# jcmgray/cotengra

Hardware: NVIDIA H100
Metric: sycamore_n53_m20_sliced_contract_tflops (higher is better)
Workload: dtype c128 (f64 arithmetic)

## Files before the change

cotengra_b200/_lib.py:

```python

from __future__ import annotations

import ctypes as C
import os

from . import lowering

_HERE = os.path.dirname(os.path.abspath(__file__))
LIB_PATH = os.path.join(_HERE, "libctgb200.so")

EXPORTS = (
    "ctgb_abi_version",
    "ctgb_desc_words",
    "ctgb_single_desc_words",
    "ctgb_last_error",
    "ctgb_device_info",
    "ctgb_contract_pair",
    "ctgb_reduce_single",
    "ctgb_plan_create",
    "ctgb_plan_set_chunk_desc",
    "ctgb_plan_set_scale_slots",
    "ctgb_plan_destroy",
    "ctgb_plan_workspace_bytes",
    "ctgb_plan_launches_per_slice",
    "ctgb_plan_strip_modes",
    "ctgb_plan_execute",
    "ctgb_plan_execute_host",
    "ctgb_launch_count",
    "ctgb_tensor_map_launches",
    "ctgb_plan_profile",
    "ctgb_plan_profile_read",
    "ctgb_probe_fp64_peaks",
    "ctgb_tc05_launch_config",
    "ctgb_dmmastream_launch_config",
)
TC05_LAUNCH_FIELDS = ("b_stat", "nb", "sa", "grid", "smem", "tm_rank", "bulk", "chunk_steps", "chunks")
DMMASTREAM_LAUNCH_FIELDS = ("nj", "rows", "grid")


class CtgbTensor(C.Structure):
    _fields_ = [
        ("kind", C.c_int32),
        ("input_index", C.c_int32),
        ("offset", C.c_int64),
        ("nbytes", C.c_int64),
        ("n_sliced", C.c_int32),
        ("slice_pos", C.POINTER(C.c_int32)),
        ("slice_stride", C.POINTER(C.c_int64)),
    ]


class CtgbNode(C.Structure):
    _fields_ = [
        ("kind", C.c_int32),
        ("a", C.c_int32),
        ("b", C.c_int32),
        ("c", C.c_int32),
        ("phase", C.c_int32),
        ("zero_fill", C.c_int32),
        ("is_root", C.c_int32),
# ... 53 lines not shown
    ]
    lib.ctgb_contract_pair.argtypes = [C.c_void_p] * 5
    lib.ctgb_reduce_single.argtypes = [C.c_void_p] * 4
    lib.ctgb_plan_create.argtypes = [C.POINTER(CtgbPlanDesc), C.POINTER(C.c_void_p)]
    lib.ctgb_plan_set_chunk_desc.argtypes = [C.c_void_p, C.c_void_p]
    lib.ctgb_plan_set_scale_slots.argtypes = [C.c_void_p, C.POINTER(C.c_int32), C.POINTER(C.c_int32), C.c_int]
    lib.ctgb_plan_destroy.argtypes = [C.c_void_p]
    lib.ctgb_plan_destroy.restype = None
    lib.ctgb_plan_execute.argtypes = [
        C.c_void_p, C.POINTER(C.c_void_p), C.c_void_p, C.c_void_p, C.c_void_p, C.POINTER(C.c_void_p),
        C.c_void_p, C.c_size_t, C.c_int64, C.c_int64, C.c_int64, C.c_void_p,
    ]
    lib.ctgb_plan_execute_host.argtypes = [
        C.c_void_p, C.POINTER(C.c_void_p), C.POINTER(C.c_int64), C.c_void_p,
        C.POINTER(C.c_double), C.c_void_p, C.c_size_t, C.c_int64, C.c_int64,
        C.c_int64, C.c_void_p,
    ]
    lib.ctgb_plan_profile.argtypes = [C.c_void_p, C.c_int]
    lib.ctgb_plan_profile_read.argtypes = [C.c_void_p, C.POINTER(C.c_float), C.c_int]
    lib.ctgb_probe_fp64_peaks.argtypes = [C.POINTER(C.c_double), C.POINTER(C.c_double), C.c_void_p]
    lib.ctgb_tc05_launch_config.argtypes = [C.c_void_p, C.c_uint64, C.c_int, C.c_uint64,
                                            C.POINTER(C.c_int64), C.c_int]
    lib.ctgb_dmmastream_launch_config.argtypes = [C.c_void_p, C.c_int, C.POINTER(C.c_int64), C.c_int]
    if lib.ctgb_abi_version() != 2:
        raise ImportError("libctgb200.so: ABI version mismatch")
    if lib.ctgb_desc_words() != lowering.DESC_WORDS:
        raise ImportError("libctgb200.so: pair descriptor layout mismatch")
    if lib.ctgb_single_desc_words() != lowering.SDESC_WORDS:
        raise ImportError("libctgb200.so: single descriptor layout mismatch")
    _lib = lib
    return lib


def check(rc):
    if rc:
        msg = load().ctgb_last_error().decode()
        raise _ERRORS.get(rc, RuntimeError)(f"ctgb error {rc}: {msg}")


def device_info():
    lib = load()
    sm, ma, mi, sh = C.c_int(), C.c_int(), C.c_int(), C.c_size_t()
    check(lib.ctgb_device_info(C.byref(sm), C.byref(ma), C.byref(mi), C.byref(sh)))
    return {"sm_count": sm.value, "cc": (ma.value, mi.value), "smem_optin": sh.value}


# ... 9 lines not shown


def tensor_map_launches() -> int:
    return int(load().ctgb_tensor_map_launches())


def tc05_launch_config(words, a_addr, sms, smem_optin) -> dict:
    import numpy as np

    w = np.ascontiguousarray(words, dtype=np.int64)
    out = (C.c_int64 * len(TC05_LAUNCH_FIELDS))()
    check(load().ctgb_tc05_launch_config(w.ctypes.data, int(a_addr), int(sms), int(smem_optin), out,
                                         len(TC05_LAUNCH_FIELDS)))
    return dict(zip(TC05_LAUNCH_FIELDS, (int(x) for x in out)))


def dmmastream_launch_config(words, sms) -> dict:
    import numpy as np

    w = np.ascontiguousarray(words, dtype=np.int64)
    out = (C.c_int64 * len(DMMASTREAM_LAUNCH_FIELDS))()
    check(load().ctgb_dmmastream_launch_config(w.ctypes.data, int(sms), out, len(DMMASTREAM_LAUNCH_FIELDS)))
    return dict(zip(DMMASTREAM_LAUNCH_FIELDS, (int(x) for x in out)))
```

cotengra_b200/csrc/ctg_b200.cu:

```cuda
#include <cuda.h>
#include <cuda_runtime.h>
#include <stdint.h>
#include <stdio.h>
#include <stdlib.h>
#include <string.h>

#include <algorithm>
#include <atomic>
#include <type_traits>
#include <string>
#include <vector>

#include "../../include/ctg_b200.h"
#include "gett_desc.h"
#include "gett_kernels.cuh"
#include "probe.cuh"

using namespace ctgb;

namespace {

thread_local std::string g_err;
std::atomic<int64_t> g_launches{0};

// ... 32 lines not shown
      cached_dev = dev;
      cudaMemPool_t pool;
      if (cudaDeviceGetDefaultMemPool(&pool, dev) == cudaSuccess) {
        uint64_t keep = UINT64_MAX;
        cudaMemPoolSetAttribute(pool, cudaMemPoolAttrReleaseThreshold, &keep);
      }
    } else {
      d.ok = false;
    }
  }
  return d;
}

size_t elem_size(int dtype) {
  switch (dtype) {
    case CTGB_F32: return 4;
    case CTGB_F64: return 8;
    case CTGB_C64: return 8;
    case CTGB_C128: return 16;
  }
  return 0;
}

template <typename T, class P>
int launch_gett_policy(const int64_t* h, const int64_t* d, const void* A, const void* B, void* C, cudaStream_t st) {
  DevInfo& di = devinfo();
  if (!di.ok) return fail(CTGB_E_CUDA, "no CUDA device");
  constexpr size_t smem = GettSmem<P>::template bytes<T>();
  if (smem > di.smem_optin) return fail(CTGB_E_CUDA, "kernel variant needs more shared memory than the device offers");
  static thread_local int attr_dev = -1;
  int dev;
  cudaGetDevice(&dev);
  if (attr_dev != dev) {
    CUDA_TRY(cudaFuncSetAttribute(gett_kernel<T, P>, cudaFuncAttributeMaxDynamicSharedMemorySize, (int)smem));
    attr_dev = dev;
  }
  if constexpr (P::CONSUMER_REGS > 0) {
    static thread_local int checked = 0;
    if (!checked) {
      cudaFuncAttributes fa;
      CUDA_TRY(cudaFuncGetAttributes(&fa, gett_kernel<T, P>));
      const long pool = (long)fa.numRegs * (P::THREADS + PRODUCER_THREADS);
      const long want = (long)P::CONSUMER_REGS * P::THREADS + (long)P::PRODUCER_REGS * PRODUCER_THREADS;
      if (want > pool) return fail(CTGB_E_CUDA, "setmaxnreg budget exceeds the launch register pool");
      checked = 1;
    }
  }
  static thread_local int occ = 0;
  if (occ == 0) {
    CUDA_TRY(cudaOccupancyMaxActiveBlocksPerMultiprocessor(&occ, gett_kernel<T, P>, P::THREADS + PRODUCER_THREADS, smem));
    if (occ < 1) occ = 1;
  }
  const uint64_t work = (uint64_t)h[W_TILES_M] * (uint64_t)h[W_TILES_N] * (uint64_t)h[W_TILES_B] * (uint64_t)h[W_SPLITK];
  if (work == 0) return CTGB_OK;
  if (work >= (1ull << 31)) return fail(CTGB_E_VALUE, "too many tiles for one launch");
  uint64_t grid = (uint64_t)di.sms * occ;
  if (grid > work) grid = work;
  if (h[W_SPLITK] > 1 && !(h[W_FLAGS] & 1)) {
    if (h[W_CELEMS] <= 0) return fail(CTGB_E_VALUE, "split-K into a strided C needs accumulate");
    CUDA_TRY(cudaMemsetAsync(C, 0, (size_t)h[W_CELEMS] * sizeof(T), st));
  }
  gett_kernel<T, P><<<(unsigned)grid, P::THREADS + PRODUCER_THREADS, smem, st>>>(d, (const T*)A, (const T*)B, (T*)C);
  g_launches.fetch_add(1, std::memory_order_relaxed);
  CUDA_TRY(cudaGetLastError());
  return CTGB_OK;
}

template <typename T>
int launch_rowstream(const int64_t* h, const int64_t* d, const void* A, const void* B, void* C, cudaStream_t st) {
  DevInfo& di = devinfo();
  if (!di.ok) return fail(CTGB_E_CUDA, "no CUDA device");
  const int N = (int)h[W_NTA], K = (int)h[W_KTA];
  if (N > 8 || K > 8 || h[W_TILES_N] != 1 || h[W_TILES_B] != 1 || h[W_STEPS_K] != 1 || h[W_SPLITK] != 1 ||
      h[W_PGM] >= 0 && (h[W_MFULL] % h[W_MTEXT]) != 0 || h[W_PGN] >= 0 || h[W_PGK] >= 0)
    return fail(CTGB_E_VALUE, "descriptor does not fit the row-stream kernel");
  const unsigned long long M = (unsigned long long)h[W_MTA] * (unsigned long long)h[W_TILES_M];
  if (M >= (1ull << 32)) return fail(CTGB_E_VALUE, "too many rows for the row-stream kernel");
  unsigned long long blocks = (M + 255) / 256;
  const unsigned long long cap = (unsigned long long)di.sms * 8;
  if (blocks > cap) blocks = cap;
  if (blocks == 0) return CTGB_OK;
  const T* a = (const T*)A;
  const T* b = (const T*)B;
  T* c = (T*)C;
  const bool strip = h[W_SCALE_A] != 0 || h[W_FACTOR_C] != 0;
  if (N <= 4 && K <= 4) {
    if (strip) rowstream_kernel<T, 4, 4, true, true><<<(unsigned)blocks, 256, 0, st>>>(d, a, b, c);
    else rowstream_kernel<T, 4, 4, true><<<(unsigned)blocks, 256, 0, st>>>(d, a, b, c);
// ... 331 lines not shown

template <typename T>
int launch_gett_typed(const int64_t* h, const int64_t* d, const void* A, const void* B, void* C, cudaStream_t st) {
  const int variant = (int)h[W_VARIANT];
  const bool one = (h[W_FLAGS] & FLAG_TF32_ONE_PASS) != 0;
  if (variant == VAR_ROWSTREAM) return launch_rowstream<T>(h, d, A, B, C, st);
  if (variant == VAR_ROWSTREAM_K) return launch_rowstream_longk<T>(h, d, A, B, C, st);
  if (variant == VAR_DMMASTREAM) return launch_dmmastream(h, d, A, B, C, st);
  if (variant == VAR_DOTSTREAM || variant == VAR_DOTSTREAM4) return launch_dotstream<T>(h, d, A, B, C, st);
  if constexpr (std::is_same<T, float2>::value) {
    if (variant == VAR_TC05_128x64) return one ? launch_tc05<64, true>(h, d, A, B, C, st) : launch_tc05<64, false>(h, d, A, B, C, st);
    if (variant == VAR_TC05_128x32) return one ? launch_tc05<32, true>(h, d, A, B, C, st) : launch_tc05<32, false>(h, d, A, B, C, st);
    if (variant == VAR_TC05_128x16) return one ? launch_tc05<16, true>(h, d, A, B, C, st) : launch_tc05<16, false>(h, d, A, B, C, st);
  }
  switch (variant) {
    case VAR_SIMT_64x64: return launch_gett_policy<T, SimtPolicy<T, 64, 64, 8, 3>>(h, d, A, B, C, st);
    case VAR_KRED: return launch_gett_policy<T, KredPolicy<T, 1, 1, 512, 6>>(h, d, A, B, C, st);
    case VAR_ROW_128x8: return launch_gett_policy<T, RowPolicy<T, 256, 8, 4, 3>>(h, d, A, B, C, st);
    case VAR_ROW_256x4: return launch_gett_policy<T, RowPolicy<T, 256, 4, 4, 3>>(h, d, A, B, C, st);
    default: break;
  }
  if constexpr (sizeof(T) == 16 || (sizeof(T) == 8 && std::is_same<T, double>::value)) {
    switch (variant) {
      case VAR_DMMA_128x64: return launch_gett_policy<T, DmmaPolicy<T, 4, 2, 4, 4, 16, 3, false, 4>>(h, d, A, B, C, st);
      case VAR_DMMA_64x128: return launch_gett_policy<T, DmmaPolicy<T, 2, 4, 4, 4, 16, 3, false, 4>>(h, d, A, B, C, st);
      case VAR_DMMA_256x32: return launch_gett_policy<T, DmmaPolicy<T, 8, 1, 4, 4, 8, 4, false, 8>>(h, d, A, B, C, st);
      case VAR_DMMA_256x16: return launch_gett_policy<T, DmmaPolicy<T, 8, 1, 4, 2, 8, 5>>(h, d, A, B, C, st);
      case VAR_DMMA_32x32: return launch_gett_policy<T, DmmaPolicy<T, 2, 2, 2, 2, 16, 4>>(h, d, A, B, C, st);
      default: break;
    }
  }
  if constexpr (sizeof(T) == 16) {
    switch (variant) {
      case VAR_DMMA3M_128x32: return launch_gett_policy<T, DmmaPolicy<T, 4, 2, 4, 2, 16, 4, true>>(h, d, A, B, C, st);
      case VAR_DMMA3M_256x16: return launch_gett_policy<T, DmmaPolicy<T, 8, 1, 4, 2, 8, 5, true>>(h, d, A, B, C, st);
      default: break;
    }
  }
  if constexpr (std::is_same<T, float>::value || std::is_same<T, float2>::value) {
    switch (variant) {
#define CTGB_TF32(...)                                                                             \
  return one ? launch_gett_policy<T, Tf32Policy<T, __VA_ARGS__, true>>(h, d, A, B, C, st)           \
             : launch_gett_policy<T, Tf32Policy<T, __VA_ARGS__>>(h, d, A, B, C, st)
      case VAR_DMMA_128x64: CTGB_TF32(4, 2, 2, 4, 16, 3);
      case VAR_DMMA_64x128: CTGB_TF32(2, 4, 2, 4, 16, 3);
      case VAR_DMMA_256x32: CTGB_TF32(8, 1, 2, 4, 8, 3);
      case VAR_DMMA_256x16: CTGB_TF32(8, 1, 2, 2, 8, 3);
      case VAR_TF32_32x32: CTGB_TF32(2, 2, 1, 2, 16, 4);
#undef CTGB_TF32
      default: break;
    }
// ... 311 lines not shown
    default: return fail(CTGB_E_VALUE, "not a wgmma descriptor");
  }
  if (rc) return rc;
  const int64_t v[9] = {lc.b_stat, lc.nb, lc.sa, (int64_t)lc.grid, (int64_t)lc.smem, lc.tm_rank, lc.bulk,
                        (int64_t)lc.chunk, (int64_t)lc.chunks};
  for (int i = 0; i < 9; ++i) out[i] = v[i];
  return CTGB_OK;
}

int ctgb_dmmastream_launch_config(const int64_t* words, int sms, int64_t* out, int n_out) {
  if (!words || !out) return fail(CTGB_E_VALUE, "null argument");
  if (words[W_MAGIC] != DESC_MAGIC) return fail(CTGB_E_VALUE, "bad descriptor");
  if (n_out < 3) return fail(CTGB_E_VALUE, "ctgb_dmmastream_launch_config writes 3 words");
  if (sms < 1) return fail(CTGB_E_VALUE, "sms must be positive");
  if (words[W_VARIANT] != VAR_DMMASTREAM) return fail(CTGB_E_VALUE, "not a DMMA stream descriptor");
  DsLaunch lc;
  if (int rc = dmmastream_launch_config(words, sms, lc)) return rc;
  out[0] = lc.nj;
  out[1] = lc.rows;
  out[2] = (int64_t)lc.blocks;
  return CTGB_OK;
}

int ctgb_device_info(int* sm_count, int* cc_major, int* cc_minor, size_t* smem_optin_bytes) {
  DevInfo& d = devinfo();
  if (!d.ok) return fail(CTGB_E_CUDA, "no CUDA device");
  if (sm_count) *sm_count = d.sms;
  if (cc_major) *cc_major = d.major;
  if (cc_minor) *cc_minor = d.minor;
  if (smem_optin_bytes) *smem_optin_bytes = d.smem_optin;
  return CTGB_OK;
}

int ctgb_probe_fp64_peaks(double* dmma_tflops, double* dfma_tflops, void* stream) {
  DevInfo& di = devinfo();
  if (!di.ok) return fail(CTGB_E_CUDA, "no CUDA device");
  cudaStream_t st = (cudaStream_t)stream;
  double* sink = nullptr;
  CUDA_TRY(cudaMalloc((void**)&sink, 64));
  cudaEvent_t e0, e1;
  CUDA_TRY(cudaEventCreate(&e0));
  CUDA_TRY(cudaEventCreate(&e1));
  const int blocks = di.sms * 8, iters = 4096;
  auto timed = [&](int which, double flop_per_thread_iter, double* out) -> int {
    float best = 1e30f;
    for (int rep = 0; rep < 4; ++rep) {
// ... 412 lines not shown
```

cotengra_b200/csrc/gett_kernels.cuh:

```cuda
#pragma once
#include <cuda_runtime.h>
#include <math_constants.h>
#include <stdint.h>

#include <type_traits>

#include "gett_desc.h"

namespace ctgb {

__device__ __forceinline__ void mac(float& c, float a, float b) { c = fmaf(a, b, c); }
__device__ __forceinline__ void mac(double& c, double a, double b) { c = fma(a, b, c); }
__device__ __forceinline__ void mac(float2& c, float2 a, float2 b) {
  c.x = fmaf(a.x, b.x, c.x);
  c.x = fmaf(-a.y, b.y, c.x);
  c.y = fmaf(a.x, b.y, c.y);
  c.y = fmaf(a.y, b.x, c.y);
}
__device__ __forceinline__ void mac(double2& c, double2 a, double2 b) {
  c.x = fma(a.x, b.x, c.x);
  c.x = fma(-a.y, b.y, c.x);
  c.y = fma(a.x, b.y, c.y);
  c.y = fma(a.y, b.x, c.y);
}
// ... 381 lines not shown

template <typename T, int WARPS_M, int WARPS_N, int FM, int FN, int KT_, int STAGES_, bool M3_ = false,
          int B_SLOTS_ = STAGES_>
struct DmmaPolicy {
  static constexpr bool CPLX = sizeof(T) == 16;
  static constexpr bool M3 = M3_ && CPLX;
  static constexpr int MT = WARPS_M * FM * 8, NT = WARPS_N * FN * 8, KT = KT_, STAGES = STAGES_;
  static constexpr int THREADS = WARPS_M * WARPS_N * 32;
  static constexpr int A_ELEMS = MT * KT, B_ELEMS = NT * KT;
  static constexpr int B_SLOTS = B_SLOTS_;
  static constexpr int SCRATCH_ELEMS = 0;
  static constexpr int CONSUMER_REGS = (THREADS == 256) ? 232 : 0, PRODUCER_REGS = 40;
  static constexpr bool HAS_BCACHE = false;
  static constexpr int MIN_BLOCKS = THREADS <= 128 ? 2 : 1;
  static_assert(KT % 4 == 0, "KT must be a multiple of the DMMA k");
  static_assert(FM % 2 == 0, "real and 3M products issue one m16n8k4 DMMA per two 8-row fragments");
  static constexpr bool TR = CPLX && !M3;
  static constexpr bool SCAN_OK = true;
  struct Acc {
    double re[FM][FN][2];
    double im[CPLX ? FM : 1][CPLX ? FN : 1][2];
    double p3[M3 ? FM : 1][M3 ? FN : 1][2];
  };
  __device__ static __forceinline__ int idxA(int r, int kk) { return ((kk >> 2) * MT + r) * 4 + (kk & 3); }
  __device__ static __forceinline__ int idxB(int c, int kk) { return ((kk >> 2) * NT + c) * 4 + (kk & 3); }
  __device__ static __forceinline__ void clear(Acc& acc) {
#pragma unroll
    for (int i = 0; i < FM; ++i)
#pragma unroll
      for (int j = 0; j < FN; ++j) {
        acc.re[i][j][0] = acc.re[i][j][1] = 0.0;
        if constexpr (CPLX) acc.im[i][j][0] = acc.im[i][j][1] = 0.0;
        if constexpr (M3) acc.p3[i][j][0] = acc.p3[i][j][1] = 0.0;
      }
  }
  __device__ static __forceinline__ void compute(const T* __restrict__ sA, const T* __restrict__ sB, Acc& acc,
                                                 int kvalid, int ncols) {
    const int lane = threadIdx.x & 31, warp = threadIdx.x >> 5;
    const int wm = warp % WARPS_M, wn = warp / WARPS_M;
    const int frow = lane >> 2, fk = lane & 3;
    const T* pa = sA + ((wm * FM * 8 + frow) * 4 + fk);
    const T* pb = sB + ((wn * FN * 8 + frow) * 4 + fk);
#pragma unroll
    for (int k4 = 0; k4 < KT / 4; ++k4) {
      if (k4 * 4 >= kvalid) break;
      T a[FM], b[FN];
#pragma unroll
      for (int i = 0; i < FM; ++i) a[i] = pa[(k4 * MT + i * 8) * 4];
#pragma unroll
      for (int j = 0; j < FN; ++j) b[j] = pb[(k4 * NT + j * 8) * 4];
      if constexpr (M3) {
        double as[FM], bs[FN];
#pragma unroll
        for (int i = 0; i < FM; ++i) as[i] = a[i].x + a[i].y;
#pragma unroll
        for (int j = 0; j < FN; ++j) bs[j] = b[j].x + b[j].y;
#pragma unroll
        for (int i = 0; i < FM; i += 2)
#pragma unroll
          for (int j = 0; j < FN; ++j) dmma16x8x4(acc.re[i][j], acc.re[i + 1][j], a[i].x, a[i + 1].x, b[j].x);
#pragma unroll
        for (int i = 0; i < FM; i += 2)
#pragma unroll
          for (int j = 0; j < FN; ++j) dmma16x8x4(acc.im[i][j], acc.im[i + 1][j], a[i].y, a[i + 1].y, b[j].y);
#pragma unroll
        for (int i = 0; i < FM; i += 2)
#pragma unroll
          for (int j = 0; j < FN; ++j) dmma16x8x4(acc.p3[i][j], acc.p3[i + 1][j], as[i], as[i + 1], bs[j]);
      } else if constexpr (CPLX) {
        double2 nb[FN];
#pragma unroll
// ... 265 lines not shown
```

cotengra_b200/csrc/gett_ws.cuh:

```cuda
#pragma once

constexpr int KCHUNK = 128;
constexpr int PRODUCER_THREADS = 128;

__device__ __forceinline__ void mbar_init(unsigned long long* bar, unsigned count) {
  unsigned a = (unsigned)__cvta_generic_to_shared(bar);
  asm volatile("mbarrier.init.shared::cta.b64 [%0], %1;\n" ::"r"(a), "r"(count) : "memory");
}
__device__ __forceinline__ void mbar_arrive(unsigned long long* bar) {
  unsigned a = (unsigned)__cvta_generic_to_shared(bar);
  asm volatile("{\n\t.reg .b64 st;\n\tmbarrier.arrive.shared::cta.b64 st, [%0];\n\t}\n" ::"r"(a) : "memory");
}
__device__ __forceinline__ void mbar_arrive_cp_async(unsigned long long* bar) {
  unsigned a = (unsigned)__cvta_generic_to_shared(bar);
  asm volatile("cp.async.mbarrier.arrive.noinc.shared::cta.b64 [%0];\n" ::"r"(a) : "memory");
}
__device__ __forceinline__ void mbar_wait(unsigned long long* bar, unsigned parity) {
  unsigned a = (unsigned)__cvta_generic_to_shared(bar);
  asm volatile(
      "{\n\t.reg .pred p;\n\t"
      "WAIT_%=:\n\t"
      "mbarrier.try_wait.parity.shared::cta.b64 p, [%0], %1;\n\t"
      "@p bra DONE_%=;\n\t"
      "bra WAIT_%=;\n\t"
// ... 12 lines not shown
template <int REGS>
__device__ __forceinline__ void reg_dealloc() {
  asm volatile("setmaxnreg.dec.sync.aligned.u32 %0;\n" ::"n"(REGS));
}

template <class P, bool HAS>
struct BCacheOf {
  struct type {};
};
template <class P>
struct BCacheOf<P, true> {
  using type = typename P::BCache;
};

template <class P, class = void>
struct BSlotsOf {
  static constexpr int value = P::STAGES;
};
template <class P>
struct BSlotsOf<P, std::void_t<decltype(P::B_SLOTS)>> {
  static constexpr int value = P::B_SLOTS > P::STAGES ? P::B_SLOTS : P::STAGES;
};

template <class P>
struct GettSmem {
  static constexpr int NA = (P::A_ELEMS + PRODUCER_THREADS - 1) / PRODUCER_THREADS;
  static constexpr int NB = (P::B_ELEMS + PRODUCER_THREADS - 1) / PRODUCER_THREADS;
  static constexpr int TI = P::STAGES + 2;
  template <typename T>
  static constexpr size_t bytes() {
    return sizeof(T) * ((size_t)P::STAGES * P::A_ELEMS + (size_t)BSlotsOf<P>::value * P::B_ELEMS +
                        P::SCRATCH_ELEMS)
           + 8 * (size_t)(NA + NB) * PRODUCER_THREADS
           + 8 * (size_t)(P::MT + P::NT)
           + 8 * (size_t)2 * KCHUNK
           + 8 * (size_t)4 * TI
           + 8 * (size_t)2 * P::STAGES
           + 4 * (size_t)(NA + NB) * PRODUCER_THREADS
           + 4 * (size_t)KCHUNK + 4 * (size_t)2 * TI
           + 64;
  }
};

template <typename T, class P>
__global__ void __launch_bounds__(P::THREADS + PRODUCER_THREADS, P::MIN_BLOCKS)
gett_kernel(const int64_t* __restrict__ D, const T* __restrict__ A, const T* __restrict__ B, T* __restrict__ C) {
  constexpr int MT = P::MT, NT = P::NT, STAGES = P::STAGES, BSLOTS = BSlotsOf<P>::value;
  constexpr int NCONS = P::THREADS, NPROD = PRODUCER_THREADS, NTHR = NCONS + NPROD;
  constexpr int NA = GettSmem<P>::NA, NB = GettSmem<P>::NB, TI = GettSmem<P>::TI;
  extern __shared__ __align__(16) unsigned char smem_raw[];
  T* sA = reinterpret_cast<T*>(smem_raw);
  T* sB = sA + STAGES * P::A_ELEMS;
  T* scratch = sB + BSLOTS * P::B_ELEMS;
  long long* gA = reinterpret_cast<long long*>(scratch + P::SCRATCH_ELEMS);
  long long* gB = gA + NA * NPROD;
  long long* offMC = gB + NB * NPROD;
  long long* offNC = offMC + MT;
  long long* kbA = offNC + NT;
  long long* kbB = kbA + KCHUNK;
  long long* ti_base = kbB + KCHUNK;
  unsigned long long* bar_full = reinterpret_cast<unsigned long long*>(ti_base + 4 * TI);
  unsigned long long* bar_empty = bar_full + STAGES;
  unsigned* metaA = reinterpret_cast<unsigned*>(bar_empty + STAGES);
  unsigned* metaB = metaA + NA * NPROD;
  int* kval = reinterpret_cast<int*>(metaB + NB * NPROD);
  int* ti_valid = kval + KCHUNK;

  const int tid = threadIdx.x;
  const int lane = tid & 31;
  const bool is_producer = tid >= NCONS;
  const int ptid = tid - NCONS;

  const int n_tm = (int)D[W_NTM], n_tn = (int)D[W_NTN];
  const int n_gm = (int)D[W_NGM], n_gn = (int)D[W_NGN], n_gk = (int)D[W_NGK], n_gb = (int)D[W_NGB];
  const int MTa = (int)D[W_MTA], NTa = (int)D[W_NTA], KTa = (int)D[W_KTA];
// ... 5 lines not shown
  const bool pair_ok = (D[W_FLAGS] & 2) != 0 && !atomic && !accumulate && sizeof(T) == 16;
  const bool ktab = steps_k <= (unsigned)KCHUNK;
  const bool g_pow2 = (D[W_FLAGS] & 4) != 0;
  auto digit_of = [&](unsigned idx, unsigned div, unsigned ext) -> unsigned {
    return g_pow2 ? ((idx >> (31 - __clz(div))) & (ext - 1)) : ((idx / div) % ext);
  };
  const bool exactA = pgm < 0 && pgk < 0, exactB = pgn < 0 && pgk < 0;

  auto kstep_bases = [&](unsigned step, long long& a, long long& b, int& kv) {
    a = 0;
    b = 0;
    kv = KTa;
    for (int j = 0; j < n_gk; ++j) {
      const int64_t* G = D + OFF_GK + j * 4;
      unsigned dig = (step / (unsigned)G[1]) % (unsigned)G[0];
      a += (long long)dig * G[2];
      b += (long long)dig * G[3];
      if (j == pgk)
        kv = (int)min((long long)D[W_KTEXT], (long long)D[W_KFULL] - (long long)dig * (long long)D[W_KTEXT]) *
             (int)D[W_KW];
    }
  };

  for (int i = tid; i < STAGES * P::A_ELEMS + BSLOTS * P::B_ELEMS; i += NTHR) sA[i] = zero_of<T>();
  if (tid == 0) {
    for (int s = 0; s < STAGES; ++s) {
      mbar_init(&bar_full[s], NPROD);
      mbar_init(&bar_empty[s], NCONS / 32);
    }
    asm volatile("fence.mbarrier_init.release.cluster;\n" ::: "memory");
  }
  if (is_producer) {
    const int n_lda = (int)D[W_NLDA], n_ldb = (int)D[W_NLDB];
    for (int i = 0; i < NA; ++i) {
      unsigned e = ptid + i * NPROD;
      long long g = 0;
      unsigned r = 0, kk = 0xFFFFu;
      if (e < (unsigned)(MTa * KTa)) {
        kk = 0;
        for (int d = 0; d < n_lda; ++d) {
          const int64_t* L = D + OFF_LDA + d * 4;
          unsigned ext = (unsigned)L[0];
          unsigned dig = e % ext;
          e /= ext;
          g += (long long)dig * L[1];
          r += dig * (unsigned)L[2];
          kk += dig * (unsigned)L[3];
        }
      }
      gA[i * NPROD + ptid] = g;
      metaA[i * NPROD + ptid] = exactA ? (kk == 0xFFFFu ? 0xFFFFFFFFu : (unsigned)P::idxA((int)r, (int)kk))
                                       : (r | (kk << 16));
    }
    for (int i = 0; i < NB; ++i) {
      unsigned e = ptid + i * NPROD;
      long long g = 0;
      unsigned c = 0, kk = 0xFFFFu;
      if (e < (unsigned)(NTa * KTa)) {
        kk = 0;
        for (int d = 0; d < n_ldb; ++d) {
          const int64_t* L = D + OFF_LDB + d * 4;
          unsigned ext = (unsigned)L[0];
          unsigned dig = e % ext;
          e /= ext;
          g += (long long)dig * L[1];
          kk += dig * (unsigned)L[2];
          c += dig * (unsigned)L[3];
        }
      }
      gB[i * NPROD + ptid] = g;
      metaB[i * NPROD + ptid] = exactB ? (kk == 0xFFFFu ? 0xFFFFFFFFu : (unsigned)P::idxB((int)c, (int)kk))
                                       : (c | (kk << 16));
    }
    if (ktab) {
      for (unsigned s = ptid; s < steps_k; s += NPROD) {
// ... 34 lines not shown
    }
  }
  __syncthreads();

  const unsigned tiles_all = tiles_m * tiles_n * tiles_b;
  const unsigned total_work = tiles_all * splitk;
  const unsigned steps_per_split = (steps_k + splitk - 1) / splitk;
  const unsigned nw = blockIdx.x < total_work ? (total_work - blockIdx.x + gridDim.x - 1) / gridDim.x : 0u;

  auto work_krange = [&](unsigned j, unsigned& k0, unsigned& k1) {
    const unsigned w = blockIdx.x + j * gridDim.x;
    const unsigned ks = w / tiles_all;
    k0 = ks * steps_per_split;
    k1 = min(steps_k, k0 + steps_per_split);
  };

  const bool b_resident = splitk == 1 && n_gb == 0 && (gridDim.x % tiles_n) == 0 && steps_k <= (unsigned)BSLOTS;
  auto b_slot = [&](unsigned step, int st) -> int { return b_resident ? (int)step : st; };

  if (is_producer) {
    if constexpr (P::CONSUMER_REGS > 0) reg_dealloc<P::PRODUCER_REGS>();
    unsigned ktab_base = 0;
    unsigned g = 0;
    for (unsigned j = 0; j < nw; ++j) {
      unsigned k0, k1;
      work_krange(j, k0, k1);
      const int slot = (int)(j % TI);
      if (ptid < 32) {
        unsigned t = blockIdx.x + j * gridDim.x;
        if (splitk > 1) t %= tiles_all;
        unsigned in_, im_, ib_;
        if (g_pow2) {
          in_ = t & (tiles_n - 1);
          t >>= 31 - __clz(tiles_n);
          im_ = t & (tiles_m - 1);
          ib_ = t >> (31 - __clz(tiles_m));
        } else {
          in_ = t % tiles_n;
          t /= tiles_n;
          im_ = t % tiles_m;
          ib_ = t / tiles_m;
        }
        long long a = 0, b = 0, c = 0;
        int vm = 0, vn = 0;
        for (int q = lane; q < n_gm; q += 32) {
          const int64_t* G = D + OFF_GM + q * 4;
// ... 34 lines not shown
          __threadfence_block();
        }
      }
      named_sync<1, NPROD>();
      const long long tA = ti_base[slot * 4 + 0], tB = ti_base[slot * 4 + 1];
      const unsigned m_valid = (unsigned)ti_valid[slot * 2 + 0], n_valid = (unsigned)ti_valid[slot * 2 + 1];

      for (unsigned step = k0; step < k1; ++step, ++g) {
        if (!ktab && (step == k0 || step >= ktab_base + KCHUNK)) {
          named_sync<1, NPROD>();
          ktab_base = step;
          for (unsigned s = ptid; s < (unsigned)KCHUNK && step + s < k1; s += NPROD) {
            long long a, b;
            int kv;
            kstep_bases(step + s, a, b, kv);
            kbA[s] = a;
            kbB[s] = b;
            kval[s] = kv;
          }
          named_sync<1, NPROD>();
        }
        const int st = (int)(g % STAGES);
        mbar_wait(&bar_empty[st], ((g / STAGES) & 1) ^ 1);
        T* dA = sA + st * P::A_ELEMS;
        T* dB = sB + b_slot(step, st) * P::B_ELEMS;
        const unsigned ti = step - ktab_base;
        const T* srcA = A + tA + kbA[ti];
        const T* srcB = B + tB + kbB[ti];
        const unsigned kv = (unsigned)kval[ti];
        if (exactA) {
#pragma unroll
          for (int i = 0; i < NA; ++i) {
            const unsigned meta = metaA[i * NPROD + ptid];
            if (meta != 0xFFFFFFFFu) cp_async_zfill<sizeof(T)>(dA + meta, srcA + gA[i * NPROD + ptid], true);
          }
        } else {
#pragma unroll
          for (int i = 0; i < NA; ++i) {
            const unsigned meta = metaA[i * NPROD + ptid];
            const unsigned r = meta & 0xFFFFu, kk = meta >> 16;
            if (kk != 0xFFFFu) {
              const bool ok = (r < m_valid) && (kk < kv);
              cp_async_zfill<sizeof(T)>(dA + P::idxA(r, kk), ok ? (srcA + gA[i * NPROD + ptid]) : A, ok);
            }
          }
        }
        if (b_resident && g >= steps_k) {
        } else if (exactB) {
#pragma unroll
          for (int i = 0; i < NB; ++i) {
            const unsigned meta = metaB[i * NPROD + ptid];
            if (meta != 0xFFFFFFFFu) cp_async_zfill<sizeof(T)>(dB + meta, srcB + gB[i * NPROD + ptid], true);
          }
// ... 22 lines not shown
    P::clear(acc);
    StripCtx sctx = strip_begin(D);
    unsigned g = 0;
    [[maybe_unused]] const bool b_invariant = steps_k == 1 && n_gn == 0 && n_gb == 0;
    [[maybe_unused]] bool b_loaded = false;
    [[maybe_unused]] typename BCacheOf<P, P::HAS_BCACHE>::type bcache;
    for (unsigned j = 0; j < nw; ++j) {
      unsigned k0, k1;
      work_krange(j, k0, k1);
      for (unsigned step = k0; step < k1; ++step, ++g) {
        const int st = (int)(g % STAGES);
        int kv = KTa;
        if (pgk >= 0) {
          const int dig = (int)((step / pk_div) % pk_ext);
          kv = min(ktext, kfull - dig * ktext) * kw;
        }
        mbar_wait(&bar_full[st], (g / STAGES) & 1);
        if constexpr (P::HAS_BCACHE) {
          if (b_invariant) {
            if (!b_loaded) {
              P::load_b(sB + b_slot(step, st) * P::B_ELEMS, bcache);
              b_loaded = true;
            }
            P::compute_cached(sA + st * P::A_ELEMS, bcache, acc, kv, NTa);
          } else {
            P::compute(sA + st * P::A_ELEMS, sB + b_slot(step, st) * P::B_ELEMS, acc, kv, NTa);
          }
        } else
          P::compute(sA + st * P::A_ELEMS, sB + b_slot(step, st) * P::B_ELEMS, acc, kv, NTa);
        __syncwarp();
        if (lane == 0) mbar_arrive(&bar_empty[st]);
      }
      const int slot = (int)(j % TI);
      const long long baseC = ti_base[slot * 4 + 2];
      const int m_valid = ti_valid[slot * 2 + 0], n_valid = ti_valid[slot * 2 + 1];
      T* const ctile = C + baseC;
      P::finalize(acc);
      bool strip_store = false;
      if (sctx.on) {
        if (sctx.scale || !P::SCAN_OK) {
          strip_store = true;
        } else {
          int hmax = 0;
          P::epilogue(
              acc, scratch, [&](int, int, T v) { hmax = max(hmax, strip_hi(v)); },
              [&](int, int, T v0, T v1) { hmax = max(hmax, max(strip_hi(v0), strip_hi(v1))); }, pair_ok, n_valid);
          if (strip_hot<T>(sctx, hmax)) {
            P::epilogue(
                acc, scratch,
                [&](int r, int c, T v) {
                  if (r < m_valid && c < n_valid) strip_note(sctx, v);
                },
// ... 73 lines not shown
```

include/ctg_b200.h:

```cpp
#ifndef CTG_B200_H
#define CTG_B200_H

#include <stddef.h>
#include <stdint.h>

#ifdef __cplusplus
extern "C" {
#endif

#define CTGB_ABI_VERSION 2

enum {
  CTGB_F32 = 0,
  CTGB_F64 = 1,
  CTGB_C64 = 2,
  CTGB_C128 = 3
};

enum {
  CTGB_OK = 0,
  CTGB_E_VALUE = 1,
  CTGB_E_NOTIMPL = 2,
  CTGB_E_CUDA = 3,
  CTGB_E_MEMORY = 4
// ... 68 lines not shown
                      size_t workspace_bytes, int64_t slice_begin,
                      int64_t slice_step, int64_t slice_count, void* stream);

int ctgb_plan_execute_host(ctgb_plan* plan, const void* const* host_inputs,
                           const int64_t* input_nbytes, void* host_out,
                           double* host_exponent, void* workspace,
                           size_t workspace_bytes, int64_t slice_begin,
                           int64_t slice_step, int64_t slice_count,
                           void* stream);

int ctgb_plan_profile(ctgb_plan* plan, int enable);
int ctgb_plan_profile_read(ctgb_plan* plan, float* ms, int n_nodes);

int ctgb_probe_fp64_peaks(double* dmma_tflops, double* dfma_tflops, void* stream);

int64_t ctgb_launch_count(void);
int64_t ctgb_tensor_map_launches(void);

int ctgb_tc05_launch_config(const int64_t* words, uint64_t a_addr, int sms,
                            uint64_t smem_optin, int64_t* out, int n_out);

int ctgb_dmmastream_launch_config(const int64_t* words, int sms, int64_t* out, int n_out);

#ifdef __cplusplus
}
#endif
#endif
```

Baseline: 21.31.

## Fill DMMA A stages with TMA bulk copies when A runs are contiguous

Adds bulk-copy variants of the 128x64 and 64x128 DMMA tiles. When the A operand's k-major layout has contiguous runs of at least 128 bytes, producer warps issue cp.async.bulk transfers completing on the stage mbarrier, replacing per-element loads. A k-major padded shared-memory A layout is used in these variants, and the ring gets 4 stages. This is meant to cut producer instruction overhead and address math, at the cost of more shared memory, a different A smem layout that may cause bank conflicts, and eligibility checks at launch time.

Result: faster. 21.83, median of 6 (+2.4%).

```diff
diff --git a/cotengra_b200/_lib.py b/cotengra_b200/_lib.py
--- a/cotengra_b200/_lib.py
+++ b/cotengra_b200/_lib.py
@@ -33,9 +33,11 @@
     "ctgb_probe_fp64_peaks",
     "ctgb_tc05_launch_config",
     "ctgb_dmmastream_launch_config",
+    "ctgb_dmma_launch_config",
 )
 TC05_LAUNCH_FIELDS = ("b_stat", "nb", "sa", "grid", "smem", "tm_rank", "bulk", "chunk_steps", "chunks")
 DMMASTREAM_LAUNCH_FIELDS = ("nj", "rows", "grid")
+DMMA_LAUNCH_FIELDS = ("run", "runs", "stages", "smem")
 
 
 class CtgbTensor(C.Structure):
@@ -135,6 +137,7 @@
     lib.ctgb_tc05_launch_config.argtypes = [C.c_void_p, C.c_uint64, C.c_int, C.c_uint64,
                                             C.POINTER(C.c_int64), C.c_int]
     lib.ctgb_dmmastream_launch_config.argtypes = [C.c_void_p, C.c_int, C.POINTER(C.c_int64), C.c_int]
+    lib.ctgb_dmma_launch_config.argtypes = [C.c_void_p, C.c_uint64, C.c_uint64, C.POINTER(C.c_int64), C.c_int]
     if lib.ctgb_abi_version() != 2:
         raise ImportError("libctgb200.so: ABI version mismatch")
     if lib.ctgb_desc_words() != lowering.DESC_WORDS:
@@ -190,3 +193,12 @@
     out = (C.c_int64 * len(DMMASTREAM_LAUNCH_FIELDS))()
     check(load().ctgb_dmmastream_launch_config(w.ctypes.data, int(sms), out, len(DMMASTREAM_LAUNCH_FIELDS)))
     return dict(zip(DMMASTREAM_LAUNCH_FIELDS, (int(x) for x in out)))
+
+
+def dmma_launch_config(words, a_addr, smem_optin) -> dict:
+    import numpy as np
+
+    w = np.ascontiguousarray(words, dtype=np.int64)
+    out = (C.c_int64 * len(DMMA_LAUNCH_FIELDS))()
+    check(load().ctgb_dmma_launch_config(w.ctypes.data, int(a_addr), int(smem_optin), out, len(DMMA_LAUNCH_FIELDS)))
+    return dict(zip(DMMA_LAUNCH_FIELDS, (int(x) for x in out)))
diff --git a/cotengra_b200/csrc/ctg_b200.cu b/cotengra_b200/csrc/ctg_b200.cu
--- a/cotengra_b200/csrc/ctg_b200.cu
+++ b/cotengra_b200/csrc/ctg_b200.cu
@@ -78,8 +78,59 @@
   return 0;
 }
 
+template <typename T> using DmmaP128x64 = DmmaPolicy<T, 4, 2, 4, 4, 16, 3, false, 4>;
+template <typename T> using DmmaP64x128 = DmmaPolicy<T, 2, 4, 4, 4, 16, 3, false, 4>;
+template <typename T> using DmmaP256x32 = DmmaPolicy<T, 8, 1, 4, 4, 8, 4, false, 8>;
+template <typename T> using DmmaP256x16 = DmmaPolicy<T, 8, 1, 4, 2, 8, 5>;
+template <typename T> using DmmaP32x32 = DmmaPolicy<T, 2, 2, 2, 2, 16, 4>;
+template <typename T> using DmmaP128x64Bulk = BulkRing<T, DmmaP128x64<T>, 4>;
+template <typename T> using DmmaP64x128Bulk = BulkRing<T, DmmaP64x128<T>, 4>;
+
+struct DmmaLaunch {
+  int run = 0;
+  int runs = 0;
+  int stages = 0;
+  size_t smem = 0;
+};
+
+template <typename T, class P, class PB = P>
+int dmma_launch_config(const int64_t* h, uint64_t a_addr, uint64_t smem_optin, DmmaLaunch& lc) {
+  lc = DmmaLaunch();
+  lc.stages = P::STAGES;
+  lc.smem = GettSmem<P>::template bytes<T>();
+  if constexpr (AStageOf<P>::bulk) {
+    const int64_t* L = h + OFF_LDA;
+    auto whole = [&](int pg, int full, int text) { return h[pg] < 0 || (h[full] % h[text]) == 0; };
+    const long long tile = h[W_MTA] * h[W_KTA];
+    if (h[W_NLDA] >= 1 && L[1] == 1 && L[2] == 1 && L[3] == 0 && L[0] * (long long)sizeof(T) >= BULK_MIN_RUN_BYTES &&
+        tile % L[0] == 0 && tile / L[0] <= (long long)GettSmem<PB>::NA * PRODUCER_THREADS &&
+        whole(W_PGM, W_MFULL, W_MTEXT) && whole(W_PGK, W_KFULL, W_KTEXT) && a_addr % 16 == 0) {
+      lc.run = (int)L[0];
+      lc.runs = (int)(tile / L[0]);
+      lc.stages = PB::STAGES;
+      lc.smem = GettSmem<PB>::template bytes<T>();
+    }
+  }
+  if (lc.smem > smem_optin) return fail(CTGB_E_CUDA, "kernel variant needs more shared memory than the device offers");
+  return CTGB_OK;
+}
+
+template <typename T>
+int dmma_launch_config_of(const int64_t* h, uint64_t a_addr, uint64_t smem_optin, DmmaLaunch& lc) {
+  switch ((int)h[W_VARIANT]) {
+    case VAR_DMMA_128x64: return dmma_launch_config<T, DmmaP128x64<T>, DmmaP128x64Bulk<T>>(h, a_addr, smem_optin, lc);
+    case VAR_DMMA_64x128: return dmma_launch_config<T, DmmaP64x128<T>, DmmaP64x128Bulk<T>>(h, a_addr, smem_optin, lc);
+    case VAR_DMMA_256x32: return dmma_launch_config<T, DmmaP256x32<T>>(h, a_addr, smem_optin, lc);
+    case VAR_DMMA_256x16: return dmma_launch_config<T, DmmaP256x16<T>>(h, a_addr, smem_optin, lc);
+    case VAR_DMMA_32x32: return dmma_launch_config<T, DmmaP32x32<T>>(h, a_addr, smem_optin, lc);
+    default: break;
+  }
+  return fail(CTGB_E_VALUE, "not a staged DMMA descriptor");
+}
+
 template <typename T, class P>
-int launch_gett_policy(const int64_t* h, const int64_t* d, const void* A, const void* B, void* C, cudaStream_t st) {
+int launch_gett_policy(const int64_t* h, const int64_t* d, const void* A, const void* B, void* C, cudaStream_t st,
+                       int a_run = 0) {
   DevInfo& di = devinfo();
   if (!di.ok) return fail(CTGB_E_CUDA, "no CUDA device");
   constexpr size_t smem = GettSmem<P>::template bytes<T>();
@@ -116,10 +167,23 @@
     if (h[W_CELEMS] <= 0) return fail(CTGB_E_VALUE, "split-K into a strided C needs accumulate");
     CUDA_TRY(cudaMemsetAsync(C, 0, (size_t)h[W_CELEMS] * sizeof(T), st));
   }
-  gett_kernel<T, P><<<(unsigned)grid, P::THREADS + PRODUCER_THREADS, smem, st>>>(d, (const T*)A, (const T*)B, (T*)C);
+  gett_kernel<T, P><<<(unsigned)grid, P::THREADS + PRODUCER_THREADS, smem, st>>>(d, (const T*)A, (const T*)B, (T*)C,
+                                                                                 a_run);
   g_launches.fetch_add(1, std::memory_order_relaxed);
   CUDA_TRY(cudaGetLastError());
   return CTGB_OK;
+}
+
+template <typename T, class P, class PB = P>
+int launch_dmma(const int64_t* h, const int64_t* d, const void* A, const void* B, void* C, cudaStream_t st) {
+  DevInfo& di = devinfo();
+  if (!di.ok) return fail(CTGB_E_CUDA, "no CUDA device");
+  DmmaLaunch lc;
+  if (int rc = dmma_launch_config<T, P, PB>(h, (uint64_t)(uintptr_t)A, di.smem_optin, lc)) return rc;
+  if constexpr (AStageOf<P>::bulk) {
+    if (lc.run > 0) return launch_gett_policy<T, PB>(h, d, A, B, C, st, lc.run);
+  }
+  return launch_gett_policy<T, P>(h, d, A, B, C, st);
 }
 
 template <typename T>
@@ -497,11 +561,11 @@
   }
   if constexpr (sizeof(T) == 16 || (sizeof(T) == 8 && std::is_same<T, double>::value)) {
     switch (variant) {
-      case VAR_DMMA_128x64: return launch_gett_policy<T, DmmaPolicy<T, 4, 2, 4, 4, 16, 3, false, 4>>(h, d, A, B, C, st);
-      case VAR_DMMA_64x128: return launch_gett_policy<T, DmmaPolicy<T, 2, 4, 4, 4, 16, 3, false, 4>>(h, d, A, B, C, st);
-      case VAR_DMMA_256x32: return launch_gett_policy<T, DmmaPolicy<T, 8, 1, 4, 4, 8, 4, false, 8>>(h, d, A, B, C, st);
-      case VAR_DMMA_256x16: return launch_gett_policy<T, DmmaPolicy<T, 8, 1, 4, 2, 8, 5>>(h, d, A, B, C, st);
-      case VAR_DMMA_32x32: return launch_gett_policy<T, DmmaPolicy<T, 2, 2, 2, 2, 16, 4>>(h, d, A, B, C, st);
+      case VAR_DMMA_128x64: return launch_dmma<T, DmmaP128x64<T>, DmmaP128x64Bulk<T>>(h, d, A, B, C, st);
+      case VAR_DMMA_64x128: return launch_dmma<T, DmmaP64x128<T>, DmmaP64x128Bulk<T>>(h, d, A, B, C, st);
+      case VAR_DMMA_256x32: return launch_dmma<T, DmmaP256x32<T>>(h, d, A, B, C, st);
+      case VAR_DMMA_256x16: return launch_dmma<T, DmmaP256x16<T>>(h, d, A, B, C, st);
+      case VAR_DMMA_32x32: return launch_dmma<T, DmmaP32x32<T>>(h, d, A, B, C, st);
       default: break;
     }
   }
@@ -859,6 +923,23 @@
   return CTGB_OK;
 }
 
+int ctgb_dmma_launch_config(const int64_t* words, uint64_t a_addr, uint64_t smem_optin, int64_t* out, int n_out) {
+  if (!words || !out) return fail(CTGB_E_VALUE, "null argument");
+  if (words[W_MAGIC] != DESC_MAGIC) return fail(CTGB_E_VALUE, "bad descriptor");
+  if (n_out < 4) return fail(CTGB_E_VALUE, "ctgb_dmma_launch_config writes 4 words");
+  DmmaLaunch lc;
+  int rc;
+  if (words[W_DTYPE] == CTGB_C128) rc = dmma_launch_config_of<double2>(words, a_addr, smem_optin, lc);
+  else if (words[W_DTYPE] == CTGB_F64) rc = dmma_launch_config_of<double>(words, a_addr, smem_optin, lc);
+  else return fail(CTGB_E_VALUE, "the staged DMMA tiles take float64 and complex128");
+  if (rc) return rc;
+  out[0] = lc.run;
+  out[1] = lc.runs;
+  out[2] = lc.stages;
+  out[3] = (int64_t)lc.smem;
+  return CTGB_OK;
+}
+
 int ctgb_device_info(int* sm_count, int* cc_major, int* cc_minor, size_t* smem_optin_bytes) {
   DevInfo& d = devinfo();
   if (!d.ok) return fail(CTGB_E_CUDA, "no CUDA device");
diff --git a/cotengra_b200/csrc/gett_kernels.cuh b/cotengra_b200/csrc/gett_kernels.cuh
--- a/cotengra_b200/csrc/gett_kernels.cuh
+++ b/cotengra_b200/csrc/gett_kernels.cuh
@@ -427,7 +427,13 @@
     double im[CPLX ? FM : 1][CPLX ? FN : 1][2];
     double p3[M3 ? FM : 1][M3 ? FN : 1][2];
   };
-  __device__ static __forceinline__ int idxA(int r, int kk) { return ((kk >> 2) * MT + r) * 4 + (kk & 3); }
+  static constexpr bool A_BULK = TR && THREADS == 256;
+  static constexpr int A_LD = A_BULK ? MT + 2 : MT;
+  static constexpr int A_STAGE = A_BULK ? KT * A_LD : A_ELEMS;
+  __device__ static __forceinline__ int idxA(int r, int kk) {
+    if constexpr (A_BULK) return kk * A_LD + r;
+    return ((kk >> 2) * MT + r) * 4 + (kk & 3);
+  }
   __device__ static __forceinline__ int idxB(int c, int kk) { return ((kk >> 2) * NT + c) * 4 + (kk & 3); }
   __device__ static __forceinline__ void clear(Acc& acc) {
 #pragma unroll
@@ -444,14 +450,14 @@
     const int lane = threadIdx.x & 31, warp = threadIdx.x >> 5;
     const int wm = warp % WARPS_M, wn = warp / WARPS_M;
     const int frow = lane >> 2, fk = lane & 3;
-    const T* pa = sA + ((wm * FM * 8 + frow) * 4 + fk);
+    const T* pa = A_BULK ? sA + (fk * A_LD + wm * FM * 8 + frow) : sA + ((wm * FM * 8 + frow) * 4 + fk);
     const T* pb = sB + ((wn * FN * 8 + frow) * 4 + fk);
 #pragma unroll
     for (int k4 = 0; k4 < KT / 4; ++k4) {
       if (k4 * 4 >= kvalid) break;
       T a[FM], b[FN];
 #pragma unroll
-      for (int i = 0; i < FM; ++i) a[i] = pa[(k4 * MT + i * 8) * 4];
+      for (int i = 0; i < FM; ++i) a[i] = A_BULK ? pa[k4 * 4 * A_LD + i * 8] : pa[(k4 * MT + i * 8) * 4];
 #pragma unroll
       for (int j = 0; j < FN; ++j) b[j] = pb[(k4 * NT + j * 8) * 4];
       if constexpr (M3) {
diff --git a/cotengra_b200/csrc/gett_ws.cuh b/cotengra_b200/csrc/gett_ws.cuh
--- a/cotengra_b200/csrc/gett_ws.cuh
+++ b/cotengra_b200/csrc/gett_ws.cuh
@@ -58,14 +58,45 @@
   static constexpr int value = P::B_SLOTS > P::STAGES ? P::B_SLOTS : P::STAGES;
 };
 
+template <class P, class = void>
+struct AStageOf {
+  static constexpr int value = P::A_ELEMS;
+  static constexpr bool bulk = false;
+};
+template <class P>
+struct AStageOf<P, std::void_t<decltype(P::A_STAGE)>> {
+  static constexpr int value = P::A_STAGE;
+  static constexpr bool bulk = P::A_BULK;
+};
+
+constexpr int BULK_MIN_RUN_BYTES = 128;
+
+template <typename T, class P, int STAGES_>
+struct BulkRing : P {
+  static_assert(AStageOf<P>::bulk, "the bulk fill needs a k-major A stage");
+  static constexpr int STAGES = STAGES_;
+  static constexpr int A_TABLE = P::A_ELEMS * (int)sizeof(T) / BULK_MIN_RUN_BYTES;
+};
+template <class P, class = void>
+struct ATableOf {
+  static constexpr int value = P::A_ELEMS;
+  static constexpr bool bulk_only = false;
+};
+template <class P>
+struct ATableOf<P, std::void_t<decltype(P::A_TABLE)>> {
+  static constexpr int value = P::A_TABLE;
+  static constexpr bool bulk_only = true;
+};
+
 template <class P>
 struct GettSmem {
-  static constexpr int NA = (P::A_ELEMS + PRODUCER_THREADS - 1) / PRODUCER_THREADS;
+  static constexpr int NA = (ATableOf<P>::value + PRODUCER_THREADS - 1) / PRODUCER_THREADS;
   static constexpr int NB = (P::B_ELEMS + PRODUCER_THREADS - 1) / PRODUCER_THREADS;
+  static constexpr int A_STAGE = AStageOf<P>::value;
   static constexpr int TI = P::STAGES + 2;
   template <typename T>
   static constexpr size_t bytes() {
-    return sizeof(T) * ((size_t)P::STAGES * P::A_ELEMS + (size_t)BSlotsOf<P>::value * P::B_ELEMS +
+    return sizeof(T) * ((size_t)P::STAGES * A_STAGE + (size_t)BSlotsOf<P>::value * P::B_ELEMS +
                         P::SCRATCH_ELEMS)
            + 8 * (size_t)(NA + NB) * PRODUCER_THREADS
            + 8 * (size_t)(P::MT + P::NT)
@@ -80,13 +111,15 @@
 
 template <typename T, class P>
 __global__ void __launch_bounds__(P::THREADS + PRODUCER_THREADS, P::MIN_BLOCKS)
-gett_kernel(const int64_t* __restrict__ D, const T* __restrict__ A, const T* __restrict__ B, T* __restrict__ C) {
+gett_kernel(const int64_t* __restrict__ D, const T* __restrict__ A, const T* __restrict__ B, T* __restrict__ C,
+            int a_run) {
   constexpr int MT = P::MT, NT = P::NT, STAGES = P::STAGES, BSLOTS = BSlotsOf<P>::value;
   constexpr int NCONS = P::THREADS, NPROD = PRODUCER_THREADS, NTHR = NCONS + NPROD;
-  constexpr int NA = GettSmem<P>::NA, NB = GettSmem<P>::NB, TI = GettSmem<P>::TI;
+  constexpr int NA = GettSmem<P>::NA, NB = GettSmem<P>::NB, TI = GettSmem<P>::TI, A_STAGE = GettSmem<P>::A_STAGE;
+  constexpr bool BULK_ONLY = ATableOf<P>::bulk_only;
   extern __shared__ __align__(16) unsigned char smem_raw[];
   T* sA = reinterpret_cast<T*>(smem_raw);
-  T* sB = sA + STAGES * P::A_ELEMS;
+  T* sB = sA + STAGES * A_STAGE;
   T* scratch = sB + BSLOTS * P::B_ELEMS;
   long long* gA = reinterpret_cast<long long*>(scratch + P::SCRATCH_ELEMS);
   long long* gB = gA + NA * NPROD;
@@ -138,7 +171,8 @@
     }
   };
 
-  for (int i = tid; i < STAGES * P::A_ELEMS + BSLOTS * P::B_ELEMS; i += NTHR) sA[i] = zero_of<T>();
+  for (int i = tid; i < STAGES * A_STAGE + BSLOTS * P::B_ELEMS; i += NTHR) sA[i] = zero_of<T>();
+  if (a_run > 0) asm volatile("fence.proxy.async.shared::cta;\n" ::: "memory");
   if (tid == 0) {
     for (int s = 0; s < STAGES; ++s) {
       mbar_init(&bar_full[s], NPROD);
@@ -149,7 +183,7 @@
   if (is_producer) {
     const int n_lda = (int)D[W_NLDA], n_ldb = (int)D[W_NLDB];
     for (int i = 0; i < NA; ++i) {
-      unsigned e = ptid + i * NPROD;
+      unsigned e = (ptid + i * NPROD) * (a_run > 0 ? (unsigned)a_run : 1u);
       long long g = 0;
       unsigned r = 0, kk = 0xFFFFu;
       if (e < (unsigned)(MTa * KTa)) {
@@ -165,8 +199,9 @@
         }
       }
       gA[i * NPROD + ptid] = g;
-      metaA[i * NPROD + ptid] = exactA ? (kk == 0xFFFFu ? 0xFFFFFFFFu : (unsigned)P::idxA((int)r, (int)kk))
-                                       : (r | (kk << 16));
+      metaA[i * NPROD + ptid] = exactA || a_run > 0
+                                    ? (kk == 0xFFFFu ? 0xFFFFFFFFu : (unsigned)P::idxA((int)r, (int)kk))
+                                    : (r | (kk << 16));
     }
     for (int i = 0; i < NB; ++i) {
       unsigned e = ptid + i * NPROD;
@@ -247,6 +282,8 @@
     if constexpr (P::CONSUMER_REGS > 0) reg_dealloc<P::PRODUCER_REGS>();
     unsigned ktab_base = 0;
     unsigned g = 0;
+    const int a_runs = a_run > 0 ? MTa * KTa / a_run : 0;
+    [[maybe_unused]] const int my_runs = a_runs > ptid ? (a_runs - ptid + NPROD - 1) / NPROD : 0;
     for (unsigned j = 0; j < nw; ++j) {
       unsigned k0, k1;
       work_krange(j, k0, k1);
@@ -327,13 +364,33 @@
         }
         const int st = (int)(g % STAGES);
         mbar_wait(&bar_empty[st], ((g / STAGES) & 1) ^ 1);
-        T* dA = sA + st * P::A_ELEMS;
+        T* dA = sA + st * A_STAGE;
         T* dB = sB + b_slot(step, st) * P::B_ELEMS;
         const unsigned ti = step - ktab_base;
         const T* srcA = A + tA + kbA[ti];
         const T* srcB = B + tB + kbB[ti];
         const unsigned kv = (unsigned)kval[ti];
-        if (exactA) {
+        if constexpr (AStageOf<P>::bulk) {
+          if (a_run > 0) {
+            const unsigned bar = (unsigned)__cvta_generic_to_shared(&bar_full[st]);
+            const unsigned run_bytes = (unsigned)a_run * (unsigned)sizeof(T);
+            if (my_runs > 0)
+              asm volatile("mbarrier.expect_tx.relaxed.cta.shared::cta.b64 [%0], %1;\n" ::"r"(bar),
+                           "r"(my_runs * run_bytes)
+                           : "memory");
+#pragma unroll
+            for (int i = 0; i < NA; ++i) {
+              if (i >= my_runs) break;
+              const unsigned dst = (unsigned)__cvta_generic_to_shared(dA + metaA[i * NPROD + ptid]);
+              asm volatile(
+                  "cp.async.bulk.shared::cluster.global.mbarrier::complete_tx::bytes [%0], [%1], %2, [%3];\n" ::"r"(dst),
+                  "l"(srcA + gA[i * NPROD + ptid]), "r"(run_bytes), "r"(bar)
+                  : "memory");
+            }
+          }
+        }
+        if (BULK_ONLY || a_run > 0) {
+        } else if (exactA) {
 #pragma unroll
           for (int i = 0; i < NA; ++i) {
             const unsigned meta = metaA[i * NPROD + ptid];
@@ -402,12 +459,12 @@
               P::load_b(sB + b_slot(step, st) * P::B_ELEMS, bcache);
               b_loaded = true;
             }
-            P::compute_cached(sA + st * P::A_ELEMS, bcache, acc, kv, NTa);
+            P::compute_cached(sA + st * A_STAGE, bcache, acc, kv, NTa);
           } else {
-            P::compute(sA + st * P::A_ELEMS, sB + b_slot(step, st) * P::B_ELEMS, acc, kv, NTa);
+            P::compute(sA + st * A_STAGE, sB + b_slot(step, st) * P::B_ELEMS, acc, kv, NTa);
           }
         } else
-          P::compute(sA + st * P::A_ELEMS, sB + b_slot(step, st) * P::B_ELEMS, acc, kv, NTa);
+          P::compute(sA + st * A_STAGE, sB + b_slot(step, st) * P::B_ELEMS, acc, kv, NTa);
         __syncwarp();
         if (lane == 0) mbar_arrive(&bar_empty[st]);
       }
diff --git a/include/ctg_b200.h b/include/ctg_b200.h
--- a/include/ctg_b200.h
+++ b/include/ctg_b200.h
@@ -114,6 +114,9 @@
 
 int ctgb_dmmastream_launch_config(const int64_t* words, int sms, int64_t* out, int n_out);
 
+int ctgb_dmma_launch_config(const int64_t* words, uint64_t a_addr, uint64_t smem_optin, int64_t* out,
+                            int n_out);
+
 #ifdef __cplusplus
 }
 #endif
```
